# li779/mitsuba-im

Hardware: AMD Instinct MI355X
Metric: Msamples/sec at 1920x1080 path-trace, max depth 8 (higher is better)
Workload: dtype f32; 1 GPU; C2: Cornell box (synthetic, 32 triangles), 1920x1080, sobol sampler, 256 spp (256 per GPU-share), maxDepth 8, rrDepth 5, box filter, 1xMI355X wavefront path tracer per GPU; one process per GPU, rows interleaved over the ranks, RCCL film reduce; parallelism=tiles1, face=C-ABI (mi_render_run)

## Files before the change

### mitsuba-im_amd/csrc/api.cpp

```cpp
#include <hip/hip_runtime.h>
#include <atomic>
#include <cmath>
#include <cstdio>
#include <cstdlib>
#include <cstring>
#include <string>
#include <vector>
#include <mutex>
#include <set>
#include "scene_host.h"
#include "queues.h"
#include "fields.h"

extern "C" {
void mi_launch_generate(const DScene &, const RenderConst &, const Queues &, const BatchDesc &, uint32_t, hipStream_t);
void mi_launch_extend(const DScene &, const Queues &, int, uint32_t, hipStream_t);
void mi_launch_shade_d(const DScene &, const RenderConst &, const Queues &, int, uint32_t, size_t, hipStream_t);
void mi_launch_shade_d_env(const DScene &, const RenderConst &, const Queues &, int, uint32_t, size_t, hipStream_t);
void mi_launch_shade_rc(const DScene &, const RenderConst &, const Queues &, int, uint32_t, size_t, hipStream_t);
void mi_launch_shade_rc_env(const DScene &, const RenderConst &, const Queues &, int, uint32_t, size_t, hipStream_t);
void mi_launch_shade_rcw(const DScene &, const RenderConst &, const Queues &, int, uint32_t, size_t, hipStream_t);
void mi_launch_shade_rcw_env(const DScene &, const RenderConst &, const Queues &, int, uint32_t, size_t, hipStream_t);
void mi_launch_shadow(const DScene &, const Queues &, uint32_t, hipStream_t);
bool mi_fused_walk(const DScene &);
// ... 718 lines not shown
        buf ^= 1;
        if (r->rc.max_depth < 0 && (depth % 4) == 0) {
            if (r->pollWords < r->grid) { if (r->pollHost) (void) hipHostFree(r->pollHost); r->pollHost = nullptr; HIPCHK(hipHostMalloc((void **) &r->pollHost, (size_t) r->grid * 4, hipHostMallocDefault)); r->pollWords = r->grid; }
            if (!r->pollEv) HIPCHK(hipEventCreateWithFlags(&r->pollEv, hipEventDisableTiming));
            HIPCHK(hipMemcpyAsync(r->pollHost, Q.count[buf], (size_t) r->grid * 4, hipMemcpyDeviceToHost, st)); HIPCHK(hipEventRecord(r->pollEv, st)); HIPCHK(hipEventSynchronize(r->pollEv));
            uint64_t alive = 0; for (uint32_t k = 0; k < r->grid; ++k) alive += r->pollHost[k];
            if (!alive) break;
        }
    }
    mark(r, 0, evUsed, st);
    HIPCHK(hipGetLastError());
    return MI_OK;
}

int mi_render_run(mi_render *r, mi_tile tile, uint32_t s0, uint32_t s1) { return mi_render_run_rows(r, tile, 1, s0, s1); }

int mi_render_run_rows(mi_render *r, mi_tile tile, uint32_t rowStride, uint32_t s0, uint32_t s1) {
    if (!r) return fail(MI_ERR_INVALID, "mi_render_run: null");
    if (rowStride == 0) return fail(MI_ERR_INVALID, "mi_render_run_rows: row stride must be >= 1");
    const mi::SceneHost &h = r->scene->h;
    if (tile.x1 <= tile.x0 || tile.y1 <= tile.y0 || tile.x1 > h.width || tile.y1 > h.height) return fail(MI_ERR_INVALID, "mi_render_run: tile outside the film");
    if (s1 < s0 || s1 > r->p.spp) return fail(MI_ERR_INVALID, "mi_render_run: sample range outside [0, spp]");
    if (r->p.sampler == MI_SAMPLER_INDEPENDENT && s1 > (1u << 24)) return fail(MI_ERR_INVALID, "mi_render_run: independent stream supports < 2^24 samples per pixel");
    HIPCHK(hipSetDevice(h.device));
    const uint32_t nrows = (tile.y1 - tile.y0 + rowStride - 1) / rowStride;
    const uint32_t npix = (tile.x1 - tile.x0) * nrows;
    uint32_t planes = r->p.planes_per_batch;
    if (!planes) { static const uint64_t target = [] { const char *v = getenv("MI355PT_BATCH_PATHS"); return v && atoll(v) > 0 ? (uint64_t) atoll(v) : (uint64_t) (64u << 20); }(); planes = (uint32_t) std::max<uint64_t>(1, target / npix); }
    if (planes > s1 - s0) planes = std::max<uint32_t>(1, s1 - s0);
    if (!r->p.planes_per_batch && s1 - s0 >= (uint32_t) r->nStreams) {
        const uint32_t total = s1 - s0, ns = (uint32_t) r->nStreams;
        uint32_t nb = (total + planes - 1) / planes; nb = (nb + ns - 1) / ns * ns;
        planes = (total + nb - 1) / nb;
    }
    uint64_t need = (uint64_t) npix * planes;
    if (need > 0xFFFFFF00ull) return fail(MI_ERR_INVALID, "mi_render_run: batch larger than 2^32 paths");
    while (need > r->poolPaths) {
        int rc = allocPool(r, need);
        if (!rc) break;
        (void) hipGetLastError(); r->poolPaths = 0;
        if (r->p.planes_per_batch || planes <= 1) return rc;
        planes = (planes + 1) / 2; need = (uint64_t) npix * planes;
    }
    size_t evUsed = 0; r->launchesAll = 0;
    HIPCHK(hipEventRecord(r->evBegin, r->stream));
    const uint32_t nBatches = (s1 - s0 + planes - 1) / planes;
    const int nPools = (int) std::min<uint32_t>((uint32_t) r->nStreams, std::max(nBatches, 1u));
    if (nPools > 1) HIPCHK(hipEventRecord(r->joinEv[0], r->stream));
    for (int i = 1; i < nPools; ++i) HIPCHK(hipStreamWaitEvent(r->poolStream(i), r->joinEv[0], 0));
    int batch = 0, lastFilmPool = -1; r->lastFieldPool = -1; r->fieldChain = nPools > 1;
    for (uint32_t s = s0; s < s1; s += planes, ++batch) {
        if (r->cancel.exchange(0)) { HIPCHK(hipDeviceSynchronize()); return fail(MI_CANCELLED, "render cancelled"); }
        const int pool = batch % nPools; hipStream_t st = r->poolStream(pool);
        BatchDesc bd{}; bd.tile = tile; bd.n_pix = npix; bd.n_planes = std::min(planes, s1 - s); bd.sample_begin = s; bd.n_paths = (uint64_t) npix * bd.n_planes; bd.list = nullptr; bd.row_stride = rowStride;
        int rc = traceBatch(r, bd, nullptr, evUsed, pool); if (rc) return rc;
        if (nPools > 1 && lastFilmPool >= 0) HIPCHK(hipStreamWaitEvent(st, r->filmDone[lastFilmPool], 0));
        mi_launch_film(h.d, r->pool(pool), bd, r->film, r->spill, st);
        if (nPools > 1) { HIPCHK(hipEventRecord(r->filmDone[pool], st)); lastFilmPool = pool; }
        r->samplesTotal += bd.n_paths;
    }
    for (int i = 1; i < nPools; ++i) { HIPCHK(hipEventRecord(r->joinEv[i], r->poolStream(i))); HIPCHK(hipStreamWaitEvent(r->stream, r->joinEv[i], 0)); }
    mark(r, 0, evUsed);
    HIPCHK(hipEventRecord(r->evEnd, r->stream));
    HIPCHK(hipStreamSynchronize(r->stream));
    HIPCHK(hipGetLastError());
    float ms = 0; HIPCHK(hipEventElapsedTime(&ms, r->evBegin, r->evEnd)); r->stats.render_ms = ms;
    r->stats.extend_ms = r->stats.shade_ms = r->stats.shadow_ms = r->stats.other_ms = 0; r->stats.extend_launches = 0;
    if (r->profiling) {
        for (size_t i = 0; i + 1 < evUsed; ++i) {
            float t = 0; if (hipEventElapsedTime(&t, r->evPool[i], r->evPool[i + 1]) != hipSuccess) continue;
            switch (r->evTag[i]) { case 1: r->stats.extend_ms += t; r->stats.extend_launches++; break; case 2: r->stats.shade_ms += t; break; case 3: r->stats.shadow_ms += t; break; default: r->stats.other_ms += t; }
        }
    }
    return MI_OK;
}

int mi_render_stats(mi_render *r, mi_stats *out) {
    if (!r || !out) return fail(MI_ERR_INVALID, "mi_render_stats: null");
    HIPCHK(hipSetDevice(r->scene->h.device));
    unsigned long long c[4] = {0, 0, 0, 0};
    if (r->q.counters) HIPCHK(hipMemcpy(c, r->q.counters, 32, hipMemcpyDeviceToHost));
    for (Queues &Q : r->qx) if (Q.counters) { unsigned long long c2[4]; HIPCHK(hipMemcpy(c2, Q.counters, 32, hipMemcpyDeviceToHost)); for (int i = 0; i < 4; ++i) c[i] += c2[i]; }
    r->stats.rays = c[0] + r->mergedRays; r->stats.shadow_rays = c[1] + r->mergedShadow; r->stats.path_length_sum = c[2] + r->mergedPathLen; r->stats.samples = r->samplesTotal + r->mergedSamples; r->stats.extend_rays = c[0]; r->stats.extend_launches_all = r->launchesAll;
    *out = r->stats; return MI_OK;
}

int mi_render_film_size(mi_render *r, int layout, uint32_t *height, uint32_t *width, uint32_t *channels, uint32_t *border) {
    if (!r || layout < 0 || layout > 2) return fail(MI_ERR_INVALID, "mi_render_film_size: bad argument");
    const mi::SceneHost &h = r->scene->h; const uint32_t b = (uint32_t) h.border;
    if (height) *height = layout == 2 ? h.height : h.height + 2 * b;
    if (width) *width = layout == 2 ? h.width : h.width + 2 * b;
    if (channels) *channels = layout == 0 ? 5 : (layout == 1 ? 4 : 3);
    if (border) *border = layout == 2 ? 0 : b;
    return MI_OK;
}
static size_t layoutFloats(mi_render *r, int layout) { uint32_t hh, ww, cc, bb; mi_render_film_size(r, layout, &hh, &ww, &cc, &bb); return (size_t) hh * ww * cc; }
int mi_render_read_film_device(mi_render *r, int layout, void *dev) {
    if (!r || !dev || layout < 0 || layout > 2) return fail(MI_ERR_INVALID, "mi_render_read_film_device: bad argument");
    const mi::SceneHost &h = r->scene->h; HIPCHK(hipSetDevice(h.device));
    mi_launch_film_layout(r->film, r->spill, (float *) dev, (int) h.width + 2 * h.border, (int) h.height + 2 * h.border, h.border, layout, r->stream);
    HIPCHK(hipStreamSynchronize(r->stream)); HIPCHK(hipGetLastError());
    return MI_OK;
}
int mi_render_read_film(mi_render *r, int layout, float *host) {
    if (!r || !host) return fail(MI_ERR_INVALID, "mi_render_read_film: null");
    int rc = mi_render_read_film_device(r, layout, r->layoutTmp); if (rc) return rc;
    HIPCHK(hipMemcpy(host, r->layoutTmp, layoutFloats(r, layout) * 4, hipMemcpyDeviceToHost));
    return MI_OK;
}

int mi_render_merge_film(mi_render *dst, mi_render *src) {
    if (!dst || !src || dst == src) return fail(MI_ERR_INVALID, "mi_render_merge_film: two different render handles are needed");
    if (dst->filmFloats != src->filmFloats) return fail(MI_ERR_INVALID, "mi_render_merge_film: the two renders have different films");
    if (dst->nFields != src->nFields || memcmp(dst->fields, src->fields, sizeof(mi_field) * dst->nFields)) return fail(MI_ERR_INVALID, "mi_render_merge_film: the two renders hold different field lists (mi_render_set_fields)");
    const int dd = dst->scene->h.device, sd = src->scene->h.device; const size_t n = dst->filmFloats;
    HIPCHK(hipSetDevice(dd));
    const float *sFilm = src->film, *sSpill = src->spill;
    if (dd != sd) {
        if (!dst->mergeTmp) HIPCHK(hipMalloc((void **) &dst->mergeTmp, 2 * n * 4));
        int can = 0; HIPCHK(hipDeviceCanAccessPeer(&can, dd, sd));
        if (can) {
            static std::mutex peerMutex; static std::set<std::pair<int, int> > enabled;
            { std::lock_guard<std::mutex> l(peerMutex);
              if (!enabled.count({dd, sd})) { hipError_t e = hipDeviceEnablePeerAccess(sd, 0); if (e != hipSuccess && e != hipErrorPeerAccessAlreadyEnabled) return fail(MI_ERR_DEVICE, std::string("hipDeviceEnablePeerAccess: ") + hipGetErrorString(e)); (void) hipGetLastError(); enabled.insert({dd, sd}); } }
            HIPCHK(hipMemcpyPeerAsync(dst->mergeTmp, dd, src->film, sd, n * 4, dst->stream));
            HIPCHK(hipMemcpyPeerAsync(dst->mergeTmp + n, dd, src->spill, sd, n * 4, dst->stream));
        } else {
            std::vector<float> host(2 * n);
            HIPCHK(hipSetDevice(sd)); HIPCHK(hipMemcpy(host.data(), src->film, n * 4, hipMemcpyDeviceToHost)); HIPCHK(hipMemcpy(host.data() + n, src->spill, n * 4, hipMemcpyDeviceToHost));
            HIPCHK(hipSetDevice(dd)); HIPCHK(hipMemcpy(dst->mergeTmp, host.data(), 2 * n * 4, hipMemcpyHostToDevice));
        }
        sFilm = dst->mergeTmp; sSpill = dst->mergeTmp + n;
    }
    mi_launch_film_add(dst->film, sFilm, n, dst->stream); mi_launch_film_add(dst->spill, sSpill, n, dst->stream);
    HIPCHK(hipStreamSynchronize(dst->stream)); HIPCHK(hipGetLastError());
    if (dst->nFields) {
        const size_t nf = dst->fieldFloats; const float *fFilm = src->fieldFilm, *fSpill = src->fieldSpill; float *stage = nullptr;
        if (dd != sd) {
            std::vector<float> host(2 * nf);
            HIPCHK(hipSetDevice(sd)); HIPCHK(hipMemcpy(host.data(), src->fieldFilm, nf * 4, hipMemcpyDeviceToHost)); HIPCHK(hipMemcpy(host.data() + nf, src->fieldSpill, nf * 4, hipMemcpyDeviceToHost));
            HIPCHK(hipSetDevice(dd)); HIPCHK(hipMalloc((void **) &stage, 2 * nf * 4));
            if (hipMemcpy(stage, host.data(), 2 * nf * 4, hipMemcpyHostToDevice) != hipSuccess) { (void) hipFree(stage); return fail(MI_ERR_DEVICE, "mi_render_merge_film: cannot stage the field film"); }
            fFilm = stage; fSpill = stage + nf;
        }
        mi_launch_film_add(dst->fieldFilm, fFilm, nf, dst->stream); mi_launch_film_add(dst->fieldSpill, fSpill, nf, dst->stream);
        hipError_t e = hipStreamSynchronize(dst->stream); if (e == hipSuccess) e = hipGetLastError();
        if (stage) (void) hipFree(stage);
        if (e != hipSuccess) return fail(MI_ERR_DEVICE, std::string("mi_render_merge_film: ") + hipGetErrorString(e));
    }
    unsigned long long c[4]; mi_stats st{};
    (void) c; if (mi_render_stats(src, &st) == MI_OK) { dst->mergedRays += st.rays; dst->mergedShadow += st.shadow_rays; dst->mergedPathLen += st.path_length_sum; dst->mergedSamples += st.samples; }
    return MI_OK;
}

int mi_render_samples(mi_render *r, const uint32_t *pairs, uint64_t n, float *outLi) {
    if (!r || !pairs || !outLi || !n) return fail(MI_ERR_INVALID, "mi_render_samples: null argument");
    const mi::SceneHost &h = r->scene->h; HIPCHK(hipSetDevice(h.device));
    for (uint64_t i = 0; i < n; ++i) if (pairs[i * 3] >= h.width || pairs[i * 3 + 1] >= h.height) return fail(MI_ERR_INVALID, "mi_render_samples: pixel outside the film");
    if (n > r->poolPaths) { int rc = allocPool(r, n); if (rc) return rc; }
    uint32_t *dList = nullptr; float *dOut = nullptr; uint32_t *dSlots = nullptr;
    HIPCHK(hipMalloc((void **) &dList, n * 12)); HIPCHK(hipMalloc((void **) &dOut, n * 12)); HIPCHK(hipMalloc((void **) &dSlots, n * 4));
    HIPCHK(hipMemcpy(dList, pairs, n * 12, hipMemcpyHostToDevice));
    std::vector<uint32_t> slots(n); for (uint64_t i = 0; i < n; ++i) slots[i] = (uint32_t) i;
    HIPCHK(hipMemcpy(dSlots, slots.data(), n * 4, hipMemcpyHostToDevice));
    BatchDesc bd{}; bd.tile = mi_tile{0, 0, h.width, h.height}; bd.n_pix = (uint32_t) n; bd.n_planes = 1; bd.sample_begin = 0; bd.n_paths = n; bd.list = dList; bd.row_stride = 1;
    size_t evUsed = 0; bool prof = r->profiling; r->profiling = false;
// ... 223 lines not shown
```

### mitsuba-im_amd/csrc/kernels_trace.hip

```cpp
#include "kernels_common.h"
#include <algorithm>
#include "trace.h"
#include "trace_fused.h"

template <int STACK, int AN, bool WIDE>
__global__ __launch_bounds__(WG) void k_extend(DScene sc, Queues q, int buf) {
    __shared__ int s_stk[(STACK > 0 ? STACK : 1) * WG];
    __shared__ f4 s_exact[STACK > 0 ? 1 : MI_PACKET_MAX * 3];
    const uint32_t tid = threadIdx.x;
    unsigned long long rays = 0;
    if (STACK == 0) packetStage(sc, s_exact);
    for (uint32_t seg = blockIdx.x; seg < q.n_seg; seg += gridDim.x) {
    const uint32_t n = q.count[buf][seg];
    const uint64_t segBase = (uint64_t) seg * q.cap;
    rays += n;
    for (uint32_t i = tid; i < n; i += WG) {
        float4 ro = q.rayO[buf][segBase + i], rd = q.rayD[buf][segBase + i];
        v3 o = V(ro.x, ro.y, ro.z), d = V(rd.x, rd.y, rd.z);
        float mint, maxt, t = 0, u = 0, v = 0; uint32_t prim = 0xFFFFFFFFu; bool hit = false; int inst = -1;
        if (clipInterval(sc, o, d, ro.w, rd.w, false, mint, maxt)) {
            if (STACK == 0) hit = packetIntersect<false, AN>(sc, (AS<true>::p4) s_exact, o, d, mint, maxt, t, prim, u, v);
            else hit = traverse<false, AN, WIDE>(sc, o, d, mint, maxt, s_stk + tid, t, prim, u, v, inst);
        }
        q.hit[segBase + i] = make_float4(t, u, v, __uint_as_float(hit ? prim : 0xFFFFFFFFu));
        if ((AN & 2) && q.hitInst) q.hitInst[segBase + i] = inst;
    }
    }
    if (tid == 0 && rays) atomicAdd(&q.counters[0], rays);
}

template <int STACK, int AN, bool WIDE>
__global__ __launch_bounds__(WG) void k_shadow(DScene sc, Queues q) {
    __shared__ int s_stk[(STACK > 0 ? STACK : 1) * WG];
    __shared__ f4 s_exact[STACK > 0 ? 1 : MI_PACKET_MAX * 3];
    const uint32_t tid = threadIdx.x;
    if (STACK == 0) packetStage(sc, s_exact);
    for (uint32_t seg = blockIdx.x; seg < q.n_seg; seg += gridDim.x) {
    const uint32_t n = q.shCount[seg];
    const uint64_t segBase = (uint64_t) seg * q.cap;
    for (uint32_t i = tid; i < n; i += WG) {
        float4 so = q.shO[segBase + i], sd = q.shD[segBase + i];
        v3 o = V(so.x, so.y, so.z), d = V(sd.x, sd.y, sd.z);
        float mint, maxt, t, u, v; uint32_t prim; bool occluded = false; int inst;
        if (clipInterval(sc, o, d, MI_EPSILON, so.w, true, mint, maxt)) {
            if (STACK == 0) occluded = packetIntersect<true, AN>(sc, (AS<true>::p4) s_exact, o, d, mint, maxt, t, prim, u, v);
            else occluded = traverse<true, AN, WIDE>(sc, o, d, mint, maxt, s_stk + tid, t, prim, u, v, inst);
        }
        if (!occluded) {
            float4 c = q.shC[segBase + i]; const uint32_t pid = __float_as_uint(sd.w);
            float4 a = q.acc[pid]; a.x += c.x; a.y += c.y; a.z += c.z; q.acc[pid] = a;
        }
    }
    }
}



template <bool WIDE>
__global__ __launch_bounds__(WG) void k_extend_f(DScene sc, Queues q, int buf, uint32_t *ticket, uint32_t thr) {
    __shared__ int s_lds[FZ_LDS_WORDS];
    fusedStage<false, WIDE>(sc, q, buf, ticket, thr, s_lds);
}
template <bool WIDE>
__global__ __launch_bounds__(WG) void k_shadow_f(DScene sc, Queues q, uint32_t *ticket, uint32_t thr) {
    __shared__ int s_lds[FZ_LDS_WORDS];
    fusedStage<true, WIDE>(sc, q, 0, ticket, thr, s_lds);
}

template <bool ANY, bool WIDE, int LS>
__global__ __launch_bounds__(WG) void k_debug_fused(DScene sc, Queues q, uint32_t *ticket, uint32_t thr, int *maxSp) {
    __shared__ int s_lds[(LS + 10) * WG];
    fusedStage<ANY, WIDE, LS, true>(sc, q, 0, ticket, thr, s_lds, maxSp);
}

__global__ __launch_bounds__(WG) void k_debug_intersect(DScene sc, const float *rays, uint64_t n, int anyHit, float *out, int *outInst) {
    __shared__ int s_stk[STACK_DEPTH * WG];
    __shared__ f4 s_exact[MI_PACKET_MAX * 3];
    if (sc.packet_n) packetStage(sc, s_exact);
    const uint64_t i = (uint64_t) blockIdx.x * WG + threadIdx.x;
    if (i >= n) return;
    const float *r = rays + i * 8;
    v3 o = V(r[0], r[1], r[2]), d = V(r[4], r[5], r[6]);
    float mint, maxt, t = 0, u = 0, v = 0; uint32_t prim = 0xFFFFFFFFu; bool hit = false; int inst = -1;
    if (clipInterval(sc, o, d, r[3], r[7], anyHit != 0, mint, maxt)) {
        if (sc.packet_n) { if (anyHit) hit = packetIntersect<true, 1>(sc, (AS<true>::p4) s_exact, o, d, mint, maxt, t, prim, u, v); else hit = packetIntersect<false, 1>(sc, (AS<true>::p4) s_exact, o, d, mint, maxt, t, prim, u, v); }
        else if (sc.bvh_wide) { if (anyHit) hit = traverse<true, 3, true>(sc, o, d, mint, maxt, s_stk + threadIdx.x, t, prim, u, v, inst); else hit = traverse<false, 3, true>(sc, o, d, mint, maxt, s_stk + threadIdx.x, t, prim, u, v, inst); }
        else if (anyHit) hit = traverse<true, 3, false>(sc, o, d, mint, maxt, s_stk + threadIdx.x, t, prim, u, v, inst);
        else hit = traverse<false, 3, false>(sc, o, d, mint, maxt, s_stk + threadIdx.x, t, prim, u, v, inst);
    }
    if (outInst) outInst[i] = hit ? inst : -1;
    out[i * 4] = t; out[i * 4 + 1] = u; out[i * 4 + 2] = v; out[i * 4 + 3] = hit ? (anyHit ? 1.0f : (float) prim) : -1.0f;
}

__global__ __launch_bounds__(WG) void k_ray_intersect(DScene sc, const float *rays, uint64_t n, mi_intersection *out) {
    __shared__ int s_stk[STACK_DEPTH * WG];
    __shared__ f4 s_exact[MI_PACKET_MAX * 3];
    if (sc.packet_n) packetStage(sc, s_exact);
    const uint64_t i = (uint64_t) blockIdx.x * WG + threadIdx.x;
    if (i >= n) return;
    const float *r = rays + i * 8;
    v3 o = V(r[0], r[1], r[2]), d = V(r[4], r[5], r[6]);
    float mint, maxt, t = 0, u = 0, v = 0; uint32_t prim = 0xFFFFFFFFu; bool hit = false; int inst = -1;
    if (clipInterval(sc, o, d, r[3], r[7], false, mint, maxt)) {
        if (sc.packet_n) hit = packetIntersect<false, 1>(sc, (AS<true>::p4) s_exact, o, d, mint, maxt, t, prim, u, v);
        else if (sc.bvh_wide) hit = traverse<false, 3, true>(sc, o, d, mint, maxt, s_stk + threadIdx.x, t, prim, u, v, inst);
        else hit = traverse<false, 3, false>(sc, o, d, mint, maxt, s_stk + threadIdx.x, t, prim, u, v, inst);
    }
    mi_intersection rec; memset(&rec, 0, sizeof(rec)); rec.valid = hit ? 1u : 0u; rec.prim = 0xFFFFFFFFu; rec.instance = -1; rec.material = -1; rec.emitter = -1;
    if (hit) {
        Tabs<false> tb; tb.shade4 = (AS<false>::p4) sc.shade; tb.materials4 = (AS<false>::p4) sc.materials; tb.emitters4 = (AS<false>::p4) sc.emitters; tb.emitter_cdf = sc.emitter_cdf; tb.area_cdf = sc.area_cdf;
        Hit h;
        if (inst >= 0) fillHitInstanced(sc, tb, sc.instances[inst], o, d, t, prim, u, v, h);
        else if (prim >= sc.n_tris) fillHitAnalytic(sc.analytic[prim - sc.n_tris], o, d, t, u, v, h);
        else fillHit<false, true>(sc, tb, d, t, prim, u, v, h);
        if (inst < 0 && prim >= sc.n_tris) { v3 du, dv; analyticUV(sc.analytic[prim - sc.n_tris], u, v, o + d * t, h.uvx, h.uvy, du, dv); }
        rec.t = t; rec.p[0] = h.p.x; rec.p[1] = h.p.y; rec.p[2] = h.p.z; rec.ng[0] = h.ng.x; rec.ng[1] = h.ng.y; rec.ng[2] = h.ng.z;
        rec.ns[0] = h.ns.x; rec.ns[1] = h.ns.y; rec.ns[2] = h.ns.z; rec.s[0] = h.s.x; rec.s[1] = h.s.y; rec.s[2] = h.s.z; rec.tt[0] = h.t.x; rec.tt[1] = h.t.y; rec.tt[2] = h.t.z;
        rec.uv[0] = h.uvx; rec.uv[1] = h.uvy; rec.wi[0] = h.wi.x; rec.wi[1] = h.wi.y; rec.wi[2] = h.wi.z; rec.bary[0] = u; rec.bary[1] = v;
        rec.prim = prim; rec.instance = inst; rec.material = h.material; rec.emitter = h.emitter;
    }
    out[i] = rec;
}

extern "C" {
static const bool kForceStack24 = getenv("MI355PT_STACK24") != nullptr;
#define MI_BY_STACK_W(KERNEL, AN, W, ...) do { \
    if (sc.bvh_depth <= 8) hipLaunchKernelGGL((KERNEL<8, AN, W>), dim3(grid), dim3(WG), 0, st, __VA_ARGS__); \
    else if (sc.bvh_depth <= 12) hipLaunchKernelGGL((KERNEL<12, AN, W>), dim3(grid), dim3(WG), 0, st, __VA_ARGS__); \
    else if (sc.bvh_depth <= 16) hipLaunchKernelGGL((KERNEL<16, AN, W>), dim3(grid), dim3(WG), 0, st, __VA_ARGS__); \
    else if (sc.bvh_depth <= 20 && !kForceStack24) hipLaunchKernelGGL((KERNEL<20, AN, W>), dim3(grid), dim3(WG), 0, st, __VA_ARGS__); \
    else if (sc.bvh_depth <= 24) hipLaunchKernelGGL((KERNEL<24, AN, W>), dim3(grid), dim3(WG), 0, st, __VA_ARGS__); \
    else if (sc.bvh_depth <= 28) hipLaunchKernelGGL((KERNEL<28, AN, W>), dim3(grid), dim3(WG), 0, st, __VA_ARGS__); \
    else hipLaunchKernelGGL((KERNEL<STACK_DEPTH, AN, W>), dim3(grid), dim3(WG), 0, st, __VA_ARGS__); } while (0)
#define MI_BY_STACK(KERNEL, AN, ...) do { \
    if (sc.packet_n) hipLaunchKernelGGL((KERNEL<0, (AN) & 1, false>), dim3(grid), dim3(WG), 0, st, __VA_ARGS__); \
    else if (sc.bvh_wide) MI_BY_STACK_W(KERNEL, AN, true, __VA_ARGS__); \
    else MI_BY_STACK_W(KERNEL, AN, false, __VA_ARGS__); } while (0)
void mi_launch_extend(const DScene &sc, const Queues &q, int buf, uint32_t grid, hipStream_t st) {
    const int mode = (sc.n_analytic ? 1 : 0) | (sc.n_instances ? 2 : 0);
    if (mode == 3) MI_BY_STACK(k_extend, 3, sc, q, buf); else if (mode == 2) MI_BY_STACK(k_extend, 2, sc, q, buf); else if (mode == 1) MI_BY_STACK(k_extend, 1, sc, q, buf); else MI_BY_STACK(k_extend, 0, sc, q, buf);
}
void mi_launch_shadow(const DScene &sc, const Queues &q, uint32_t grid, hipStream_t st) {
    const int mode = (sc.n_analytic ? 1 : 0) | (sc.n_instances ? 2 : 0);
    if (mode == 3) MI_BY_STACK(k_shadow, 3, sc, q); else if (mode == 2) MI_BY_STACK(k_shadow, 2, sc, q); else if (mode == 1) MI_BY_STACK(k_shadow, 1, sc, q); else MI_BY_STACK(k_shadow, 0, sc, q);
}
#undef MI_BY_STACK
#undef MI_BY_STACK_W
static const int kFused = [] { const char *e = getenv("MI355PT_FUSED"); return e && e[0] ? atoi(e) : 1; }();
static const uint32_t kFusedThr = [] { const char *e = getenv("MI355PT_FUSED_THR"); const int v = e && e[0] ? atoi(e) : 48; return (uint32_t) (v < 1 ? 1 : (v > 64 ? 64 : v)); }();
static const uint32_t kFusedGrid = [] { const char *e = getenv("MI355PT_FUSED_GRID"); const int v = e && e[0] ? atoi(e) : 1792; return (uint32_t) (v < 1 ? 1 : (v > 16384 ? 16384 : v)); }();
bool mi_fused_walk(const DScene &sc) { return kFused && (sc.bvh_wide || kFused == 2) && !sc.packet_n && !sc.n_analytic && !sc.n_instances && sc.geo_bytes < 0xFFFFFF00ull; }
uint32_t mi_fused_grid(void) { return kFusedGrid; }
void mi_launch_extend_fused(const DScene &sc, const Queues &q, int buf, uint32_t *ticket, hipStream_t st) {
    const uint32_t g = kFusedGrid;
    if (sc.bvh_wide) hipLaunchKernelGGL((k_extend_f<true>), dim3(g), dim3(WG), 0, st, sc, q, buf, ticket, kFusedThr); else hipLaunchKernelGGL((k_extend_f<false>), dim3(g), dim3(WG), 0, st, sc, q, buf, ticket, kFusedThr);
}
void mi_launch_shadow_fused(const DScene &sc, const Queues &q, uint32_t *ticket, hipStream_t st) {
    const uint32_t g = kFusedGrid;
    if (sc.bvh_wide) hipLaunchKernelGGL((k_shadow_f<true>), dim3(g), dim3(WG), 0, st, sc, q, ticket, kFusedThr); else hipLaunchKernelGGL((k_shadow_f<false>), dim3(g), dim3(WG), 0, st, sc, q, ticket, kFusedThr);
}
void mi_launch_debug_fused(const DScene &sc, const Queues &q, int anyHit, uint32_t ldsStack, uint32_t *ticket, uint32_t thr, uint32_t grid, int *maxSp, hipStream_t st) {
#define MI_DBG_FUSED(ANY, WIDE) do { \
    if (ldsStack == 4u) hipLaunchKernelGGL((k_debug_fused<ANY, WIDE, 4>), dim3(grid), dim3(WG), 0, st, sc, q, ticket, thr, maxSp); \
    else hipLaunchKernelGGL((k_debug_fused<ANY, WIDE, FZ_LDS_STACK>), dim3(grid), dim3(WG), 0, st, sc, q, ticket, thr, maxSp); } while (0)
    if (anyHit) { if (sc.bvh_wide) MI_DBG_FUSED(true, true); else MI_DBG_FUSED(true, false); }
    else { if (sc.bvh_wide) MI_DBG_FUSED(false, true); else MI_DBG_FUSED(false, false); }
#undef MI_DBG_FUSED
}
uint32_t mi_fused_lds_stack(void) { return FZ_LDS_STACK; }
void mi_launch_ray_intersect(const DScene &sc, const float *rays, uint64_t n, mi_intersection *out, hipStream_t st) { hipLaunchKernelGGL(k_ray_intersect, dim3((unsigned) ((n + WG - 1) / WG)), dim3(WG), 0, st, sc, rays, n, out); }
void mi_launch_debug_intersect(const DScene &sc, const float *rays, uint64_t n, int anyHit, float *out, int *outInst, hipStream_t st) { hipLaunchKernelGGL(k_debug_intersect, dim3((unsigned) ((n + WG - 1) / WG)), dim3(WG), 0, st, sc, rays, n, anyHit, out, outInst); }
}
```

### mitsuba-im_amd/csrc/trace.h

```cpp
#pragma once
#include "kernels_common.h"

DEV bool slab(f4 lo, f4 hi, v3 inv, v3 oi, float tmin, float tmax, float &tnear) {
    float ax = __builtin_fmaf(lo.x, inv.x, oi.x), bx = __builtin_fmaf(hi.x, inv.x, oi.x);
    float ay = __builtin_fmaf(lo.y, inv.y, oi.y), by = __builtin_fmaf(hi.y, inv.y, oi.y);
    float az = __builtin_fmaf(lo.z, inv.z, oi.z), bz = __builtin_fmaf(hi.z, inv.z, oi.z);
    float t0 = fmaxf(fmaxf(fminf(ax, bx), fminf(ay, by)), fmaxf(fminf(az, bz), tmin));
    float t1 = fminf(fminf(fmaxf(ax, bx), fmaxf(ay, by)), fminf(fmaxf(az, bz), tmax));
    tnear = t0;
    return t0 <= t1 * 1.000002f + 1e-30f;
}
DEV bool aabbRay(const float *lo, const float *hi, v3 o, v3 d, float &nearT, float &farT) {
    float nt = -INFINITY, ft = INFINITY;
    const float oo[3] = {o.x, o.y, o.z}, dd[3] = {d.x, d.y, d.z};
#pragma unroll
    for (int i = 0; i < 3; ++i) {
        float origin = oo[i], minv = lo[i], maxv = hi[i], di = dd[i];
        if (di == 0) { if (origin < minv || origin > maxv) return false; }
        else {
            float rcp = 1.0f / di;
            float t1 = (minv - origin) * rcp, t2 = (maxv - origin) * rcp;
            if (t1 > t2) { float tmp = t1; t1 = t2; t2 = tmp; }
            nt = maxf(t1, nt); ft = minf(t2, ft);
            if (!(nt <= ft)) return false;
// ... 58 lines not shown
                    const uint32_t more = (key[1] != 0xFFFFFFFFu) + (key[2] != 0xFFFFFFFFu) + (key[3] != 0xFFFFFFFFu);
                    if (more) { stk[sp * WG] = (int) ((uint32_t) cur | ((key[1] & 3u) << 23) | ((key[2] & 3u) << 25) | ((key[3] & 3u) << 27) | ((more - 1u) << 29)); ++sp; }
                    cur = childOf(key[0]);
                }
            }
        } else
        while (cur >= 0 && cur != BVH_DONE) {
            f4 n0 = nodes4[cur * 4 + 0], n1 = nodes4[cur * 4 + 1], n2 = nodes4[cur * 4 + 2], n3 = nodes4[cur * 4 + 3];
            int c0 = __float_as_int(n0.w), c1 = __float_as_int(n1.w);
            float t0, t1;
            const float far = (AN & 2) ? fminf(best, cap) : best;
            bool h0 = slab(n0, n1, inv, oi, mint, far, t0), h1 = slab(n2, n3, inv, oi, mint, far, t1);
            if (h0 && h1) {
                bool swap = t1 < t0;
                stk[sp * WG] = swap ? c0 : c1; ++sp;
                cur = swap ? c1 : c0;
            } else if (h0) cur = c0;
            else if (h1) cur = c1;
            else BVH_POP();
        }
        if (cur == BVH_DONE) break;
        {
            uint32_t code = (uint32_t) ~cur; uint32_t first = code >> 3, cnt = (code & 7u) + 1u;
            bool entered = false;
            for (uint32_t i = 0; i < cnt; ++i) {
                f4 a = tris4[(first + i) * 3 + 0], b = tris4[(first + i) * 3 + 1], c = tris4[(first + i) * 3 + 2];
                TriAccelD ta; ta.k = __float_as_uint(a.x); ta.n_u = a.y; ta.n_v = a.z; ta.n_d = a.w;
                ta.a_u = b.x; ta.a_v = b.y; ta.b_nu = b.z; ta.b_nv = b.w; ta.c_nu = c.x; ta.c_nv = c.y; ta.prim = __float_as_uint(c.z);
                float u, v, t; bool ok;
                if ((AN & 2) && ta.k == MI_K_INSTANCE) {
                    const InstanceD &in = sc.instances[ta.prim];
                    v3 o2 = xfPoint(in.to_object, o0), d2 = xfVector(in.to_object, d0);
                    float nearT, farT;
                    if (aabbRay(in.glo, in.ghi, o2, d2, nearT, farT)) {
                        const float mi = mint0 > nearT ? mint0 : nearT, ma = best < farT ? best : farT;
                        if (ma > mi) {
                            stk[sp * WG] = BVH_RET; ++sp;
                            o = o2; d = d2; mint = mi; cap = farT; curInst = (int) ta.prim;
                            inv = V(safeInv(d.x), safeInv(d.y), safeInv(d.z)); oi = V(-o.x * inv.x, -o.y * inv.y, -o.z * inv.z);
                            cur = in.root; entered = true;
                        }
                    }
                    break;
                }
                const float far = (AN & 2) ? fminf(best, cap) : best;
                if ((AN & 1) && ta.k == MI_K_ANALYTIC) ok = analyticIntersect<ANY>(sc.analytic[ta.prim - sc.n_tris], o, d, mint, far, t, u, v);
                else ok = triIntersect(ta, o, d, mint, far, u, v, t);
                if (ok) {
                    if (ANY) return true;
                    if (!found || t < best || (t == best && (ta.prim < bprim || (ta.prim == bprim && curInst < binst)))) { best = t; bprim = ta.prim; binst = curInst; bu = u; bv = v; found = true; }
                }
            }
            if (!entered) BVH_POP();
        }
    }
#undef BVH_POP
    bestT = best; bestPrim = bprim; bestU = bu; bestV = bv; bestInst = binst;
    return found;
}

typedef const __attribute__((address_space(4))) f4 *cf4p;
struct PacketGroupS { f4 g0, g1, g2; };
typedef const __attribute__((address_space(4))) PacketGroupS *cgrp;
template <typename MaskT> DEV MaskT maskBit(uint32_t p) { return p < sizeof(MaskT) * 8u ? (MaskT) 1 << p : (MaskT) 0; }
template <int K, typename MaskT>
DEV void packetPass1(cgrp g, uint32_t count, v3 o, v3 d, float mint, float maxt, float so1e5, MaskT &mask) {
    const float o_u = K == 0 ? o.y : (K == 1 ? o.z : o.x), o_v = K == 0 ? o.z : (K == 1 ? o.x : o.y), o_k = K == 0 ? o.x : (K == 1 ? o.y : o.z);
    const float d_u = K == 0 ? d.y : (K == 1 ? d.z : d.x), d_v = K == 0 ? d.z : (K == 1 ? d.x : d.y), d_k = K == 0 ? d.x : (K == 1 ? d.y : d.z);
    for (; count; --count, ++g) {
        const f4 g0 = g->g0, g1 = g->g1, g2 = g->g2;
        const MaskT bit0 = maskBit<MaskT>(__float_as_uint(g2.z)), bit1 = maskBit<MaskT>(__float_as_uint(g2.w));
        const float D = __builtin_fmaf(d_u, g0.x, __builtin_fmaf(d_v, g0.y, d_k));
        const float N = __builtin_fmaf(-o_v, g0.y, __builtin_fmaf(-o_u, g0.x, g0.z - o_k));
        const float r = __builtin_amdgcn_rcpf(D), t = N * r, q = fabsf(r) + 1.0f;
        const float mt = q * __builtin_fmaf(fabsf(t), 2e-6f, so1e5);
        const float hu = __builtin_fmaf(t, d_u, o_u - g0.w), hv = __builtin_fmaf(t, d_v, o_v - g1.x);
        const float u = __builtin_fmaf(hv, g1.y, hu * g1.z), v = __builtin_fmaf(hu, g1.w, hv * g2.x);
        const float m = g2.y * mt, s = u + v, one = 1.0f + m;
        const bool reject = (fabsf(D) >= 1e-4f) & ((t + mt < mint) | (t - mt > maxt) | (s < -m) | (s > one) | (v < -m) | (v > one));
        mask |= (reject | (u < -m)) ? (MaskT) 0 : bit0;
        mask |= (reject | (u > m)) ? (MaskT) 0 : bit1;
    }
}
template <bool ANY, int AN, typename MaskT>
DEV bool packetIntersectM(const DScene &sc, AS<true>::p4 s_exact, v3 o, v3 d, float mint, float maxt, float &bestT, uint32_t &bestPrim, float &bestU, float &bestV) {
    float best = maxt; uint32_t bprim = 0xFFFFFFFFu; bool found = false; float bu = 0, bv = 0;
    MaskT mask = 0;
    const float so1e5 = maxf(maxf(sc.packet_scale, fabsf(o.x)), maxf(fabsf(o.y), fabsf(o.z))) * 1e-5f;
    cgrp groups = (cgrp) sc.packet_groups;
    packetPass1<0, MaskT>(groups, sc.packet_gk[0], o, d, mint, maxt, so1e5, mask);
    packetPass1<1, MaskT>(groups + sc.packet_gk[0], sc.packet_gk[1] - sc.packet_gk[0], o, d, mint, maxt, so1e5, mask);
    packetPass1<2, MaskT>(groups + sc.packet_gk[1], sc.packet_gk[2] - sc.packet_gk[1], o, d, mint, maxt, so1e5, mask);
    while (mask) {
        const uint32_t i = sizeof(MaskT) == 8 ? (uint32_t) __builtin_ctzll((unsigned long long) mask) : (uint32_t) __builtin_ctz((uint32_t) mask); mask &= mask - 1;
        const f4 a = s_exact[i * 3u], b = s_exact[i * 3u + 1u], c = s_exact[i * 3u + 2u];
        const bool k0 = __float_as_uint(a.x) == 0u, k1 = __float_as_uint(a.x) == 1u;
        const float o_u = k0 ? o.y : (k1 ? o.z : o.x), o_v = k0 ? o.z : (k1 ? o.x : o.y), o_k = k0 ? o.x : (k1 ? o.y : o.z);
        const float d_u = k0 ? d.y : (k1 ? d.z : d.x), d_v = k0 ? d.z : (k1 ? d.x : d.y), d_k = k0 ? d.x : (k1 ? d.y : d.z);
        const float tt = (a.w - o_u * a.y - o_v * a.z - o_k) / (d_u * a.y + d_v * a.z + d_k);
        const float hu = o_u + tt * d_u - b.x, hv = o_v + tt * d_v - b.y;
        const float uu = hv * b.z + hu * b.w, vv = hu * c.x + hv * c.y;
        const bool ok = !(tt < mint) & !(tt > best) & (uu >= 0) & (vv >= 0) & (uu + vv <= 1.0f);
        if (ANY) { found |= ok; mask = ok ? (MaskT) 0 : mask; }
        else {
            const bool better = ok & (!found | (tt < best));
            best = better ? tt : best; bprim = better ? i : bprim; bu = better ? uu : bu; bv = better ? vv : bv; found |= ok;
        }
    }
    if (ANY && found) return true;
    if (AN & 1) {
        for (uint32_t i = 0; i < sc.n_analytic; ++i) {
            AnalyticD sh;
            { cf4p src = (cf4p) (sc.analytic + i); f4 *dst = reinterpret_cast<f4 *>(&sh);
#pragma unroll
              for (int j = 0; j < 10; ++j) dst[j] = src[j]; }
            float u, v, t; const uint32_t prim = sc.n_tris + i;
            if (analyticIntersect<ANY>(sh, o, d, mint, best, t, u, v)) {
                if (ANY) return true;
                if (!found || t < best || prim < bprim) { best = t; bprim = prim; bu = u; bv = v; found = true; }
            }
        }
    }
    bestT = best; bestPrim = bprim; bestU = bu; bestV = bv;
    return found;
}
template <bool ANY, int AN>
DEV bool packetIntersect(const DScene &sc, AS<true>::p4 s_exact, v3 o, v3 d, float mint, float maxt, float &bestT, uint32_t &bestPrim, float &bestU, float &bestV) {
    if (sc.n_tris <= 32u) return packetIntersectM<ANY, AN, uint32_t>(sc, s_exact, o, d, mint, maxt, bestT, bestPrim, bestU, bestV);
    return packetIntersectM<ANY, AN, unsigned long long>(sc, s_exact, o, d, mint, maxt, bestT, bestPrim, bestU, bestV);
}
DEV void packetStage(const DScene &sc, f4 *s_exact) {
    const f4 *src = reinterpret_cast<const f4 *>(sc.packet_exact);
    for (uint32_t i = threadIdx.x; i < sc.n_tris * 3u; i += blockDim.x) s_exact[i] = src[i];
    __syncthreads();
}
```

Measured before the change: 3252 Msamples/s.

## Redistribute packet exact triangle tests across wave lanes via LDS work ring

Result: slower. 3107 Msamples/s (-4.5%).

```diff
diff --git a/mitsuba-im_amd/csrc/api.cpp b/mitsuba-im_amd/csrc/api.cpp
--- a/mitsuba-im_amd/csrc/api.cpp
+++ b/mitsuba-im_amd/csrc/api.cpp
@@ -824,6 +824,9 @@
     if (r->q.counters) HIPCHK(hipMemcpy(c, r->q.counters, 32, hipMemcpyDeviceToHost));
     for (Queues &Q : r->qx) if (Q.counters) { unsigned long long c2[4]; HIPCHK(hipMemcpy(c2, Q.counters, 32, hipMemcpyDeviceToHost)); for (int i = 0; i < 4; ++i) c[i] += c2[i]; }
     r->stats.rays = c[0] + r->mergedRays; r->stats.shadow_rays = c[1] + r->mergedShadow; r->stats.path_length_sum = c[2] + r->mergedPathLen; r->stats.samples = r->samplesTotal + r->mergedSamples; r->stats.extend_rays = c[0]; r->stats.extend_launches_all = r->launchesAll;
+#ifdef MI_PACKET_COUNT
+    r->stats.extend_rays = c[3];
+#endif
     *out = r->stats; return MI_OK;
 }
 
diff --git a/mitsuba-im_amd/csrc/kernels_trace.hip b/mitsuba-im_amd/csrc/kernels_trace.hip
--- a/mitsuba-im_amd/csrc/kernels_trace.hip
+++ b/mitsuba-im_amd/csrc/kernels_trace.hip
@@ -3,55 +3,92 @@
 #include "trace.h"
 #include "trace_fused.h"
 
+#ifdef MI_PACKET_COUNT
+#define PK_DBG_DECL unsigned long long dbgCount = 0;
+#define PK_DBG_FLUSH(WHICH) if ((MI_PACKET_COUNT == WHICH || MI_PACKET_COUNT == WHICH + 2) && (threadIdx.x & 63u) == 0 && dbgCount) { atomicAdd(reinterpret_cast<unsigned int *>(&q.counters[3]), (unsigned int) dbgCount); atomicAdd(reinterpret_cast<unsigned int *>(&q.counters[3]) + 1, (unsigned int) (dbgCount >> 32)); }
+#else
+#define PK_DBG_DECL
+#define PK_DBG_FLUSH(WHICH)
+#endif
+
 template <int STACK, int AN, bool WIDE>
 __global__ __launch_bounds__(WG) void k_extend(DScene sc, Queues q, int buf) {
     __shared__ int s_stk[(STACK > 0 ? STACK : 1) * WG];
     __shared__ f4 s_exact[STACK > 0 ? 1 : MI_PACKET_MAX * 3];
+    __shared__ __attribute__((aligned(16))) uint32_t s_wave[STACK > 0 ? 1 : PK_WAVE_WORDS * (WG / 64)];
     const uint32_t tid = threadIdx.x;
     unsigned long long rays = 0;
+    PK_DBG_DECL
     if (STACK == 0) packetStage(sc, s_exact);
     for (uint32_t seg = blockIdx.x; seg < q.n_seg; seg += gridDim.x) {
     const uint32_t n = q.count[buf][seg];
     const uint64_t segBase = (uint64_t) seg * q.cap;
     rays += n;
+    if (STACK == 0) {
+        for (uint32_t base = tid & ~63u; base < n; base += WG) {
+            const uint32_t i = base + (tid & 63u); const bool valid = i < n;
+            float4 ro = make_float4(0, 0, 0, 0), rd = make_float4(0, 0, 0, 0);
+            if (valid) { ro = q.rayO[buf][segBase + i]; rd = q.rayD[buf][segBase + i]; }
+            v3 o = V(ro.x, ro.y, ro.z), d = V(rd.x, rd.y, rd.z);
+            float mint = 0, maxt = 0, t = 0, u = 0, v = 0; uint32_t prim = 0xFFFFFFFFu;
+            const bool inside = valid && clipInterval(sc, o, d, ro.w, rd.w, false, mint, maxt);
+            bool hit = false;
+            if (__ballot(inside) != 0ull) hit = packetIntersect<false, AN>(sc, (AS<true>::p4) s_exact, (lds_w32) s_wave + (tid >> 6) * PK_WAVE_WORDS, inside, o, d, mint, maxt, t, prim, u, v PK_DBG_ARG);
+            if (valid) q.hit[segBase + i] = inside ? make_float4(t, u, v, __uint_as_float(hit ? prim : 0xFFFFFFFFu)) : make_float4(0.0f, 0.0f, 0.0f, __uint_as_float(0xFFFFFFFFu));
+        }
+    } else
     for (uint32_t i = tid; i < n; i += WG) {
         float4 ro = q.rayO[buf][segBase + i], rd = q.rayD[buf][segBase + i];
         v3 o = V(ro.x, ro.y, ro.z), d = V(rd.x, rd.y, rd.z);
         float mint, maxt, t = 0, u = 0, v = 0; uint32_t prim = 0xFFFFFFFFu; bool hit = false; int inst = -1;
-        if (clipInterval(sc, o, d, ro.w, rd.w, false, mint, maxt)) {
-            if (STACK == 0) hit = packetIntersect<false, AN>(sc, (AS<true>::p4) s_exact, o, d, mint, maxt, t, prim, u, v);
-            else hit = traverse<false, AN, WIDE>(sc, o, d, mint, maxt, s_stk + tid, t, prim, u, v, inst);
-        }
+        if (clipInterval(sc, o, d, ro.w, rd.w, false, mint, maxt)) hit = traverse<false, AN, WIDE>(sc, o, d, mint, maxt, s_stk + tid, t, prim, u, v, inst);
         q.hit[segBase + i] = make_float4(t, u, v, __uint_as_float(hit ? prim : 0xFFFFFFFFu));
         if ((AN & 2) && q.hitInst) q.hitInst[segBase + i] = inst;
     }
     }
     if (tid == 0 && rays) atomicAdd(&q.counters[0], rays);
+    PK_DBG_FLUSH(1)
 }
 
 template <int STACK, int AN, bool WIDE>
 __global__ __launch_bounds__(WG) void k_shadow(DScene sc, Queues q) {
     __shared__ int s_stk[(STACK > 0 ? STACK : 1) * WG];
     __shared__ f4 s_exact[STACK > 0 ? 1 : MI_PACKET_MAX * 3];
+    __shared__ __attribute__((aligned(16))) uint32_t s_wave[STACK > 0 ? 1 : PK_WAVE_WORDS * (WG / 64)];
     const uint32_t tid = threadIdx.x;
+    PK_DBG_DECL
     if (STACK == 0) packetStage(sc, s_exact);
     for (uint32_t seg = blockIdx.x; seg < q.n_seg; seg += gridDim.x) {
     const uint32_t n = q.shCount[seg];
     const uint64_t segBase = (uint64_t) seg * q.cap;
+    if (STACK == 0) {
+        for (uint32_t base = tid & ~63u; base < n; base += WG) {
+            const uint32_t i = base + (tid & 63u); const bool valid = i < n;
+            float4 so = make_float4(0, 0, 0, 0), sd = make_float4(0, 0, 0, 0);
+            if (valid) { so = q.shO[segBase + i]; sd = q.shD[segBase + i]; }
+            v3 o = V(so.x, so.y, so.z), d = V(sd.x, sd.y, sd.z);
+            float mint = 0, maxt = 0, t, u, v; uint32_t prim;
+            const bool inside = valid && clipInterval(sc, o, d, MI_EPSILON, so.w, true, mint, maxt);
+            bool occluded = false;
+            if (__ballot(inside) != 0ull) occluded = packetIntersect<true, AN>(sc, (AS<true>::p4) s_exact, (lds_w32) s_wave + (tid >> 6) * PK_WAVE_WORDS, inside, o, d, mint, maxt, t, prim, u, v PK_DBG_ARG);
+            if (valid && !occluded) {
+                float4 c = q.shC[segBase + i]; const uint32_t pid = __float_as_uint(sd.w);
+                float4 a = q.acc[pid]; a.x += c.x; a.y += c.y; a.z += c.z; q.acc[pid] = a;
+            }
+        }
+    } else
     for (uint32_t i = tid; i < n; i += WG) {
         float4 so = q.shO[segBase + i], sd = q.shD[segBase + i];
         v3 o = V(so.x, so.y, so.z), d = V(sd.x, sd.y, sd.z);
         float mint, maxt, t, u, v; uint32_t prim; bool occluded = false; int inst;
-        if (clipInterval(sc, o, d, MI_EPSILON, so.w, true, mint, maxt)) {
-            if (STACK == 0) occluded = packetIntersect<true, AN>(sc, (AS<true>::p4) s_exact, o, d, mint, maxt, t, prim, u, v);
-            else occluded = traverse<true, AN, WIDE>(sc, o, d, mint, maxt, s_stk + tid, t, prim, u, v, inst);
-        }
+        if (clipInterval(sc, o, d, MI_EPSILON, so.w, true, mint, maxt)) occluded = traverse<true, AN, WIDE>(sc, o, d, mint, maxt, s_stk + tid, t, prim, u, v, inst);
         if (!occluded) {
             float4 c = q.shC[segBase + i]; const uint32_t pid = __float_as_uint(sd.w);
             float4 a = q.acc[pid]; a.x += c.x; a.y += c.y; a.z += c.z; q.acc[pid] = a;
         }
     }
     }
+    PK_DBG_FLUSH(2)
 }
 
 
@@ -76,15 +113,24 @@
 __global__ __launch_bounds__(WG) void k_debug_intersect(DScene sc, const float *rays, uint64_t n, int anyHit, float *out, int *outInst) {
     __shared__ int s_stk[STACK_DEPTH * WG];
     __shared__ f4 s_exact[MI_PACKET_MAX * 3];
+    __shared__ __attribute__((aligned(16))) uint32_t s_wave[PK_WAVE_WORDS * (WG / 64)];
+    PK_DBG_DECL
     if (sc.packet_n) packetStage(sc, s_exact);
     const uint64_t i = (uint64_t) blockIdx.x * WG + threadIdx.x;
-    if (i >= n) return;
-    const float *r = rays + i * 8;
+    const bool valid = i < n;
+    if (!valid && !sc.packet_n) return;
+    float r[8] = {0, 0, 0, 0, 0, 0, 0, 0};
+    if (valid) for (int j = 0; j < 8; ++j) r[j] = rays[i * 8 + j];
     v3 o = V(r[0], r[1], r[2]), d = V(r[4], r[5], r[6]);
-    float mint, maxt, t = 0, u = 0, v = 0; uint32_t prim = 0xFFFFFFFFu; bool hit = false; int inst = -1;
-    if (clipInterval(sc, o, d, r[3], r[7], anyHit != 0, mint, maxt)) {
-        if (sc.packet_n) { if (anyHit) hit = packetIntersect<true, 1>(sc, (AS<true>::p4) s_exact, o, d, mint, maxt, t, prim, u, v); else hit = packetIntersect<false, 1>(sc, (AS<true>::p4) s_exact, o, d, mint, maxt, t, prim, u, v); }
-        else if (sc.bvh_wide) { if (anyHit) hit = traverse<true, 3, true>(sc, o, d, mint, maxt, s_stk + threadIdx.x, t, prim, u, v, inst); else hit = traverse<false, 3, true>(sc, o, d, mint, maxt, s_stk + threadIdx.x, t, prim, u, v, inst); }
+    float mint = 0, maxt = 0, t = 0, u = 0, v = 0; uint32_t prim = 0xFFFFFFFFu; bool hit = false; int inst = -1;
+    const bool inside = valid && clipInterval(sc, o, d, r[3], r[7], anyHit != 0, mint, maxt);
+    if (sc.packet_n) {
+        const lds_w32 wave = (lds_w32) s_wave + (threadIdx.x >> 6) * PK_WAVE_WORDS;
+        if (__ballot(inside) != 0ull) { if (anyHit) hit = packetIntersect<true, 1>(sc, (AS<true>::p4) s_exact, wave, inside, o, d, mint, maxt, t, prim, u, v PK_DBG_ARG); else hit = packetIntersect<false, 1>(sc, (AS<true>::p4) s_exact, wave, inside, o, d, mint, maxt, t, prim, u, v PK_DBG_ARG); }
+        if (!inside) { t = 0; hit = false; }
+        if (!valid) return;
+    } else if (inside) {
+        if (sc.bvh_wide) { if (anyHit) hit = traverse<true, 3, true>(sc, o, d, mint, maxt, s_stk + threadIdx.x, t, prim, u, v, inst); else hit = traverse<false, 3, true>(sc, o, d, mint, maxt, s_stk + threadIdx.x, t, prim, u, v, inst); }
         else if (anyHit) hit = traverse<true, 3, false>(sc, o, d, mint, maxt, s_stk + threadIdx.x, t, prim, u, v, inst);
         else hit = traverse<false, 3, false>(sc, o, d, mint, maxt, s_stk + threadIdx.x, t, prim, u, v, inst);
     }
@@ -95,15 +141,23 @@
 __global__ __launch_bounds__(WG) void k_ray_intersect(DScene sc, const float *rays, uint64_t n, mi_intersection *out) {
     __shared__ int s_stk[STACK_DEPTH * WG];
     __shared__ f4 s_exact[MI_PACKET_MAX * 3];
+    __shared__ __attribute__((aligned(16))) uint32_t s_wave[PK_WAVE_WORDS * (WG / 64)];
+    PK_DBG_DECL
     if (sc.packet_n) packetStage(sc, s_exact);
     const uint64_t i = (uint64_t) blockIdx.x * WG + threadIdx.x;
-    if (i >= n) return;
-    const float *r = rays + i * 8;
+    const bool valid = i < n;
+    if (!valid && !sc.packet_n) return;
+    float r[8] = {0, 0, 0, 0, 0, 0, 0, 0};
+    if (valid) for (int j = 0; j < 8; ++j) r[j] = rays[i * 8 + j];
     v3 o = V(r[0], r[1], r[2]), d = V(r[4], r[5], r[6]);
-    float mint, maxt, t = 0, u = 0, v = 0; uint32_t prim = 0xFFFFFFFFu; bool hit = false; int inst = -1;
-    if (clipInterval(sc, o, d, r[3], r[7], false, mint, maxt)) {
-        if (sc.packet_n) hit = packetIntersect<false, 1>(sc, (AS<true>::p4) s_exact, o, d, mint, maxt, t, prim, u, v);
-        else if (sc.bvh_wide) hit = traverse<false, 3, true>(sc, o, d, mint, maxt, s_stk + threadIdx.x, t, prim, u, v, inst);
+    float mint = 0, maxt = 0, t = 0, u = 0, v = 0; uint32_t prim = 0xFFFFFFFFu; bool hit = false; int inst = -1;
+    const bool inside = valid && clipInterval(sc, o, d, r[3], r[7], false, mint, maxt);
+    if (sc.packet_n) {
+        if (__ballot(inside) != 0ull) hit = packetIntersect<false, 1>(sc, (AS<true>::p4) s_exact, (lds_w32) s_wave + (threadIdx.x >> 6) * PK_WAVE_WORDS, inside, o, d, mint, maxt, t, prim, u, v PK_DBG_ARG);
+        if (!inside) hit = false;
+        if (!valid) return;
+    } else if (inside) {
+        if (sc.bvh_wide) hit = traverse<false, 3, true>(sc, o, d, mint, maxt, s_stk + threadIdx.x, t, prim, u, v, inst);
         else hit = traverse<false, 3, false>(sc, o, d, mint, maxt, s_stk + threadIdx.x, t, prim, u, v, inst);
     }
     mi_intersection rec; memset(&rec, 0, sizeof(rec)); rec.valid = hit ? 1u : 0u; rec.prim = 0xFFFFFFFFu; rec.instance = -1; rec.material = -1; rec.emitter = -1;
diff --git a/mitsuba-im_amd/csrc/trace.h b/mitsuba-im_amd/csrc/trace.h
--- a/mitsuba-im_amd/csrc/trace.h
+++ b/mitsuba-im_amd/csrc/trace.h
@@ -164,8 +164,45 @@
         mask |= (reject | (u > m)) ? (MaskT) 0 : bit1;
     }
 }
+#define PK_RING 128
+#define PK_WAVE_WORDS (12 * 64 + 2 * 64 + PK_RING)
+#ifndef MI_PACKET_COOP_MIN
+#define MI_PACKET_COOP_MIN 5
+#endif
+typedef __attribute__((address_space(3))) uint32_t *lds_w32;
+typedef __attribute__((address_space(3))) float *lds_wf;
+typedef __attribute__((address_space(3))) unsigned long long *lds_w64;
+DEV void waveLdsFence() { __builtin_amdgcn_fence(__ATOMIC_RELEASE, "wavefront"); __builtin_amdgcn_wave_barrier(); __builtin_amdgcn_fence(__ATOMIC_ACQUIRE, "wavefront"); }
+DEV bool packetExactLds(AS<true>::p4 s_exact, lds_wf ray, uint32_t src, uint32_t tri, float &tt, float &uu, float &vv) {
+    const f4 a = s_exact[tri * 3u], b = s_exact[tri * 3u + 1u], c = s_exact[tri * 3u + 2u];
+    const lds_wf r = ray + (__float_as_uint(a.x) * 64u + src);
+    const float o_k = r[0], o_u = r[64], o_v = r[128], d_k = r[320], d_u = r[384], d_v = r[448];
+    const float mint = ray[640u + src], maxt = ray[704u + src];
+    tt = (a.w - o_u * a.y - o_v * a.z - o_k) / (d_u * a.y + d_v * a.z + d_k);
+    const float hu = o_u + tt * d_u - b.x, hv = o_v + tt * d_v - b.y;
+    uu = hv * b.z + hu * b.w; vv = hu * c.x + hv * c.y;
+    return !(tt < mint) & !(tt > maxt) & (uu >= 0) & (vv >= 0) & (uu + vv <= 1.0f);
+}
+template <bool ANY>
+DEV void packetCoopRound(AS<true>::p4 s_exact, lds_wf ray, lds_w64 keys, lds_w32 ring, uint32_t first, uint32_t cnt, uint32_t lane) {
+    if (lane < cnt) {
+        const uint32_t e = ring[(first + lane) & (PK_RING - 1u)], src = e >> 8, tri = e & 0xFFu;
+        float tt, uu, vv;
+        if (packetExactLds(s_exact, ray, src, tri, tt, uu, vv)) {
+            if (ANY) keys[src] = 0ull;
+            else {
+                const uint32_t tr = __float_as_uint(tt), tb = tr == 0x80000000u ? 0u : tr, ord = tb ^ ((uint32_t) ((int32_t) tb >> 31) | 0x80000000u);
+                (void) __hip_atomic_fetch_min(keys + src, ((unsigned long long) ord << 32) | tri, __ATOMIC_RELAXED, __HIP_MEMORY_SCOPE_WORKGROUP);
+            }
+        }
+    }
+}
 template <bool ANY, int AN, typename MaskT>
-DEV bool packetIntersectM(const DScene &sc, AS<true>::p4 s_exact, v3 o, v3 d, float mint, float maxt, float &bestT, uint32_t &bestPrim, float &bestU, float &bestV) {
+DEV bool packetIntersectM(const DScene &sc, AS<true>::p4 s_exact, lds_w32 wave, bool active, v3 o, v3 d, float mint, float maxt, float &bestT, uint32_t &bestPrim, float &bestU, float &bestV
+#ifdef MI_PACKET_COUNT
+                          , unsigned long long &dbgCount
+#endif
+                          ) {
     float best = maxt; uint32_t bprim = 0xFFFFFFFFu; bool found = false; float bu = 0, bv = 0;
     MaskT mask = 0;
     const float so1e5 = maxf(maxf(sc.packet_scale, fabsf(o.x)), maxf(fabsf(o.y), fabsf(o.z))) * 1e-5f;
@@ -173,6 +210,51 @@
     packetPass1<0, MaskT>(groups, sc.packet_gk[0], o, d, mint, maxt, so1e5, mask);
     packetPass1<1, MaskT>(groups + sc.packet_gk[0], sc.packet_gk[1] - sc.packet_gk[0], o, d, mint, maxt, so1e5, mask);
     packetPass1<2, MaskT>(groups + sc.packet_gk[1], sc.packet_gk[2] - sc.packet_gk[1], o, d, mint, maxt, so1e5, mask);
+    mask = active ? mask : (MaskT) 0;
+    MaskT deep = mask;
+#pragma unroll
+    for (int j = 1; j < MI_PACKET_COOP_MIN; ++j) deep &= deep - 1;
+    const bool coop = __ballot(deep != 0) != 0ull;
+#ifdef MI_PACKET_COUNT
+    {
+        uint32_t c = sizeof(MaskT) == 8 ? (uint32_t) __popcll((unsigned long long) mask) : (uint32_t) __popc((uint32_t) mask), mx = c, sum = c;
+        for (int s = 1; s < 64; s <<= 1) { mx = max(mx, (uint32_t) __shfl_xor((int) mx, s)); sum += (uint32_t) __shfl_xor((int) sum, s); }
+        dbgCount += MI_PACKET_COUNT <= 2 ? ((unsigned long long) sum << 32) | mx : ((unsigned long long) (coop ? 1u : 0u) << 32) | 1u;
+    }
+#endif
+    if (coop) {
+        const uint32_t lane = threadIdx.x & 63u;
+        const lds_wf ray = (lds_wf) wave; const lds_w64 keys = (lds_w64) (wave + 12 * 64); const lds_w32 ring = wave + 14 * 64;
+        waveLdsFence();
+        ray[lane] = o.x; ray[64u + lane] = o.y; ray[128u + lane] = o.z; ray[192u + lane] = o.x; ray[256u + lane] = o.y;
+        ray[320u + lane] = d.x; ray[384u + lane] = d.y; ray[448u + lane] = d.z; ray[512u + lane] = d.x; ray[576u + lane] = d.y;
+        ray[640u + lane] = mint; ray[704u + lane] = maxt;
+        keys[lane] = ~0ull;
+        uint32_t head = 0, tail = 0;
+        unsigned long long have;
+        while ((have = __ballot(mask != 0)) != 0ull) {
+            if (mask != 0) {
+                const uint32_t i = sizeof(MaskT) == 8 ? (uint32_t) __builtin_ctzll((unsigned long long) mask) : (uint32_t) __builtin_ctz((uint32_t) mask); mask &= mask - 1;
+                const uint32_t pos = head + __builtin_amdgcn_mbcnt_hi((uint32_t) (have >> 32), __builtin_amdgcn_mbcnt_lo((uint32_t) have, 0u));
+                ring[pos & (PK_RING - 1u)] = (lane << 8) | i;
+            }
+            head += (uint32_t) __popcll(have);
+            if (head - tail >= 64u) {
+                waveLdsFence();
+                packetCoopRound<ANY>(s_exact, ray, keys, ring, tail, 64u, lane);
+                tail += 64u;
+                waveLdsFence();
+            }
+        }
+        waveLdsFence();
+        if (head != tail) packetCoopRound<ANY>(s_exact, ray, keys, ring, tail, head - tail, lane);
+        waveLdsFence();
+        const unsigned long long key = keys[lane];
+        if (key != ~0ull) {
+            found = true;
+            if (!ANY) { float tt, uu, vv; bprim = (uint32_t) key & 0xFFu; packetExactLds(s_exact, ray, lane, bprim, tt, uu, vv); best = tt; bu = uu; bv = vv; }
+        }
+    } else
     while (mask) {
         const uint32_t i = sizeof(MaskT) == 8 ? (uint32_t) __builtin_ctzll((unsigned long long) mask) : (uint32_t) __builtin_ctz((uint32_t) mask); mask &= mask - 1;
         const f4 a = s_exact[i * 3u], b = s_exact[i * 3u + 1u], c = s_exact[i * 3u + 2u];
@@ -190,7 +272,7 @@
         }
     }
     if (ANY && found) return true;
-    if (AN & 1) {
+    if ((AN & 1) && active) {
         for (uint32_t i = 0; i < sc.n_analytic; ++i) {
             AnalyticD sh;
             { cf4p src = (cf4p) (sc.analytic + i); f4 *dst = reinterpret_cast<f4 *>(&sh);
@@ -206,10 +288,17 @@
     bestT = best; bestPrim = bprim; bestU = bu; bestV = bv;
     return found;
 }
+#ifdef MI_PACKET_COUNT
+#define PK_DBG_PARAM , unsigned long long &dbgCount
+#define PK_DBG_ARG , dbgCount
+#else
+#define PK_DBG_PARAM
+#define PK_DBG_ARG
+#endif
 template <bool ANY, int AN>
-DEV bool packetIntersect(const DScene &sc, AS<true>::p4 s_exact, v3 o, v3 d, float mint, float maxt, float &bestT, uint32_t &bestPrim, float &bestU, float &bestV) {
-    if (sc.n_tris <= 32u) return packetIntersectM<ANY, AN, uint32_t>(sc, s_exact, o, d, mint, maxt, bestT, bestPrim, bestU, bestV);
-    return packetIntersectM<ANY, AN, unsigned long long>(sc, s_exact, o, d, mint, maxt, bestT, bestPrim, bestU, bestV);
+DEV bool packetIntersect(const DScene &sc, AS<true>::p4 s_exact, lds_w32 wave, bool active, v3 o, v3 d, float mint, float maxt, float &bestT, uint32_t &bestPrim, float &bestU, float &bestV PK_DBG_PARAM) {
+    if (sc.n_tris <= 32u) return packetIntersectM<ANY, AN, uint32_t>(sc, s_exact, wave, active, o, d, mint, maxt, bestT, bestPrim, bestU, bestV PK_DBG_ARG);
+    return packetIntersectM<ANY, AN, unsigned long long>(sc, s_exact, wave, active, o, d, mint, maxt, bestT, bestPrim, bestU, bestV PK_DBG_ARG);
 }
 DEV void packetStage(const DScene &sc, f4 *s_exact) {
     const f4 *src = reinterpret_cast<const f4 *>(sc.packet_exact);
```
